# Pablete1234/parquet-floor

Measured on AMD Instinct MI355X. Metric: decoded GB/s + rows/s (node), lineitem-shape Snappy+dict, 1/2/4/8 GPUs, higher is better.
Workload: dtype u8; 1 GPU; lineitem SF1 x1 (6001215 rows x 1, 16 cols, 6 row groups of 1Mi rows), Snappy + dictionary, device-resident; row_groups_per_rank=6, compressed_page_bytes_rank0=217870360

## Files before the change

### parquet-floor_amd/csrc/pf_internal.h

```cpp
#pragma once
#include <stdint.h>

#ifdef __HIPCC__
#define PF_HD __host__ __device__
#else
#define PF_HD
#endif

namespace pf {

struct Int2 {
    int x, y;
};

struct PfOpts {
    int exec = 5;
    bool ba_fused = true;
    bool page_null = false;
    int null_stagger = 0;
    bool nest_timeout = false;
    uint32_t null_dcap = 0;
    unsigned debug_skip = 0;
    int force_serial = 0;
    int force_redo = 0;
    bool zc = true;
    bool dl_kernel = true;
    bool h2d_kernel = false;
    int h2d_grid = 256;
    bool dl_stream = true;
    bool dl_prio = false;
    bool debug_plan = false;
    int64_t nest_seg = 0;
    bool nest_seg_set = false;
    bool dbp_par = true;
    bool bloom_first = true;
    int fix_shift = 1;
};

constexpr uint32_t FBLK = 4096;
constexpr uint32_t BA_TILE = 8192;
constexpr uint64_t BA_SHORT = 48;
constexpr uint32_t STICKY_DICT = 64u << 10;
constexpr uint32_t SNAP_RB = 128;
constexpr uint32_t SNAP_WIN = 64 * SNAP_RB;
constexpr uint32_t SNAP_WWORDS = SNAP_WIN / 32;
constexpr uint32_t SNAP_BLOCK = 65536;

struct SnapWin {
    uint32_t entry;
    uint32_t exit;
    uint32_t out;
    uint32_t flags;
};

struct SnapEnt {
    uint32_t pos;
    uint32_t out;
};

enum : int32_t {
    PG_V2 = 1,
    PG_COMPRESSED = 2,
    PG_DICT = 4,
};

struct SnappyJob {
    const uint8_t* src;
    uint8_t* dst;
    uint32_t src_len;
    uint32_t dst_len;
    int32_t page;
    int32_t chunk;
    uint32_t split_base;
    uint32_t n_pieces;
    uint32_t* tokmap;
    uint32_t win_base;
    uint32_t n_win;
    uint8_t* ddst;
    uint32_t dlo;
    uint32_t dgran;
    uint32_t dflags;
    uint32_t lit;
};

struct ZstdJob {
    const uint8_t* src;
    uint8_t* dst;
    uint32_t src_len;
    uint32_t dst_len;
    int32_t page;
    int32_t chunk;
    uint32_t exact;
    uint32_t produced;
};
constexpr int ZSTD_GRID = 512;
constexpr uint32_t ZSTD_LIT_MAX = 128u << 10;
PF_HD inline uint32_t zstd_lit_stride(uint32_t max_dst) {
    return ((max_dst < ZSTD_LIT_MAX ? max_dst : ZSTD_LIT_MAX) + 255u) / 256u * 256u + 256u;
}

enum : int32_t { DONE_FIXED = 1, DONE_FLAT = 2, DONE_NULL = 4, DONE_PAGE = 8 };

enum : int32_t { DIRECT_NONE = 0, DIRECT_VALUES = 1, DIRECT_INPLACE = 2 };

struct DevPage {
    const uint8_t* body;
    const uint8_t* lvl;
    uint32_t body_len;
    uint32_t rep_len;
    uint32_t def_len;
    int32_t chunk;
    int32_t flags;
    int32_t encoding;
    int32_t def_enc;
    int32_t rep_enc;
    int32_t num_values;
    int32_t done;
    int64_t entry_start;
    int64_t n_slots;
    int64_t n_values;
    int64_t n_rows;
    int64_t n_chars;
    int64_t slot_start;
    int64_t value_start;
    int64_t row_start;
    int64_t char_start;
    uint32_t* aux;
    int64_t aux_cap;
    int32_t ba_job;
    int32_t counted;
    uint32_t* runtab;
    uint32_t* lvltab;
    uint32_t lvl_cap;
    uint64_t* dx;
    int64_t dx_total;
    int64_t dx_bad;
    uint32_t dx_data;
    uint32_t dx_pad;
    const int* jfb;
    int32_t direct;
    int32_t direct_pad;
    uint8_t* seg;
    int32_t nseg;
    int32_t seg_len;
    int32_t seg_ok;
    int32_t nwin;
    struct WinPub* npub;
    uint8_t* dbp;
    struct WinPub* dbp_pub;
    int32_t dbp_nwin;
    int32_t dbp_ok;
    uint32_t dbp_bcap;
    uint32_t dbp_pad;
};
// ... 160 lines not shown
```

### parquet-floor_amd/csrc/pf_launch.h

```cpp
#pragma once
#include <hip/hip_runtime.h>

#include "pf_internal.h"
#include "pfloor.h"

namespace pf {

void launch_snappy_serial(const SnappyJob* d_jobs, int n_jobs, const int* d_fallback, DevChunkResult* d_res, hipStream_t s);
void launch_snappy_parse(const SnappyJob* d_jobs, int n_jobs, const int2* d_wins, int n_wins, SnapWin* d_win, SnapEnt* d_ent,
                         uint32_t* d_lane_out, uint32_t* d_splits, int* d_fb, int max_nwin, hipStream_t s);
void launch_snappy_exec(const SnappyJob* d_jobs, int n_jobs, const int2* d_pieces, int n_pieces, uint32_t* d_splits, int* d_fb,
                        DevChunkResult* d_res, int exec, hipStream_t s);
void launch_snappy(const SnappyJob* d_jobs, int n_jobs, const int2* d_wins, int n_wins, SnapWin* d_win, SnapEnt* d_ent,
                   uint32_t* d_lane_out, const int2* d_pieces, int n_pieces, uint32_t* d_splits, int* d_fb,
                   DevChunkResult* d_res, int max_nwin, int exec, hipStream_t s);

void launch_zstd(ZstdJob* d_jobs, const int* d_order, int n_jobs, uint8_t* d_lit, uint32_t lit_stride, DevChunkResult* d_res,
                 hipStream_t s);

void launch_snappy_head(SnappyJob* d_jobs, int n_jobs, DevPage* d_pages, const DevChunk* d_chunks, int* d_fb,
                        const DevChunkResult* d_res, hipStream_t st);
void launch_snappy_litcopy(const SnappyJob* d_jobs, const int* d_list, int n, const int* d_fb, hipStream_t st);

void launch_ba(BaJob* d_jobs, int n_jobs, const int2* d_tiles, int n_tiles, DevChunkResult* d_res, hipStream_t st,
               bool short_values);

void launch_runs(const DevChunk* d_chunks, DevPage* d_pages, const int* d_list, int n, DevChunkResult* d_res, hipStream_t st);
void launch_lvl(const DevChunk* d_chunks, DevPage* d_pages, const int* d_list, int n, DevChunkResult* d_res, hipStream_t st,
                bool page_null, NullCaps nc);
void launch_count_flat(const DevChunk* d_chunks, DevPage* d_pages, const int* d_list, int n, int n_flat, const int2* d_dblk,
                       int n_dblk, DevChunkResult* d_res, BaJob* d_bajobs, hipStream_t st);
void launch_flat(const DevChunk* d_chunks, DevPage* d_pages, const int* d_list, int nfix, int n, int n4, int n8, int* d_fbq,
                 DevChunkResult* d_res, hipStream_t st, NullCaps nc, int stagger);

void launch_nest_lvl(const DevChunk* d_chunks, DevPage* d_pages, const int* d_list, int n, int max_nwin, DevChunkResult* d_res,
                     hipStream_t st, bool force_timeout);
void launch_count(const DevChunk* d_chunks, DevPage* d_pages, const int* d_list, int n, DevChunkResult* d_res, BaJob* d_bajobs,
                  hipStream_t st, int idle_grid);
void launch_nest_count(const DevChunk* d_chunks, DevPage* d_pages, const int* d_list, int n, const int2* d_segs, int n_segs,
                       DevChunkResult* d_res, hipStream_t st);
void launch_scan(DevChunk* d_chunks, DevPage* d_pages, const int* d_list, int n, DevChunkResult* d_res, uint8_t* arena,
                 uint64_t cap, unsigned long long* used, hipStream_t st);
void launch_decode(const DevChunk* d_chunks, DevPage* d_pages, const int* d_list, int n, int n_first, DevChunkResult* d_res,
                   hipStream_t st, int idle_grid);
void launch_nest_decode(const DevChunk* d_chunks, DevPage* d_pages, const int2* d_segs, int n_segs, DevChunkResult* d_res,
                        hipStream_t st);

void launch_delta(const DevChunk* d_chunks, DevPage* d_pages, const int* d_list, int n, int max_dbp_nwin, DevChunkResult* d_res,
                  hipStream_t st);
void launch_dlen(const DevChunk* d_chunks, DevPage* d_pages, const int* d_list, int n, DevChunkResult* d_res, hipStream_t st);
void launch_dba_chars(const DevChunk* d_chunks, DevPage* d_pages, const int* d_list, int n, DevChunkResult* d_res, hipStream_t st);

void launch_window(const DevChunk* d_chunks, const DevChunkResult* d_res, const DevWin* d_wins, DevWinRes* d_wres, int n_wins,
                   int copy_grid, const uint8_t* chars_base, uint8_t* wchars_base, int64_t out_delta, int64_t bits_delta,
                   hipStream_t st);

struct SelBufs {
    DevSelHead* head;
    DevSelChunk* sc;
    const DevPred* preds;
    const uint8_t* blob;
    const int32_t* win_of;
    uint64_t* mask;
    uint32_t* tile_count;
    uint32_t* tile_base;
    int32_t* rows;
    uint32_t* ba_sum;
    uint32_t* ba_base;
    int64_t* ba_total;
    int64_t rows_cap, tiles_cap;
    int32_t n_preds;
};
void launch_filter(const DevChunk* d_chunks, const DevChunkResult* d_res, const DevWinRes* d_wres, const SelBufs& f, int n_chunks,
                   int gather_grid, const uint8_t* chars_base, uint8_t* wchars_base, int64_t out_delta, int64_t bits_delta,
                   hipStream_t st);

void launch_page_scan(const ScanChunk* d_chunks, int n_chunks, pf_page_desc* d_pages, ScanCrc* d_crcs, ScanResult* d_res,
                      hipStream_t s);
void launch_page_crc(const ScanCrc* d_crcs, const int* d_list, int n, ScanResult* d_res, int32_t* d_bad, hipStream_t s);

}
```

### parquet-floor_amd/csrc/pf_pages.hip

```cpp
#include <hip/hip_runtime.h>

#include "pf_launch.h"
#include "pf_pages.h"
#include "pf_snappy_par.h"

namespace pf {

#ifdef PF_STAMPS
__device__ unsigned long long pf_pstamps[16];
#define PSTAMP(i, v) atomicAdd(&pf_pstamps[i], (unsigned long long)(v))
extern "C" int pf_debug_pstamps(unsigned long long* out, int n, int reset) {
    if (hipMemcpyFromSymbol(out, HIP_SYMBOL(pf_pstamps), sizeof(unsigned long long) * (n < 16 ? n : 16)) != hipSuccess) return -1;
    if (reset) {
        unsigned long long z[16] = {};
        if (hipMemcpyToSymbol(HIP_SYMBOL(pf_pstamps), z, sizeof z) != hipSuccess) return -1;
    }
    return 0;
}
#else
#define PSTAMP(i, v) ((void)0)
#endif

#ifndef PF_FT
#define PF_FT 2048
#endif
constexpr int FT = PF_FT;
constexpr int FEPT = FT / NT;
static_assert(FT <= int(FBLK) && FBLK % FT == 0 && FEPT <= 32, "tiles divide blocks; a thread's entries fit a 32-bit mask");
#ifndef PF_FTX
#define PF_FTX 2048
#endif
constexpr int FTX = PF_FTX;
constexpr int FEPTX = FTX / NT;
static_assert(FTX <= int(FBLK) && FBLK % FTX == 0, "fixed-width tiles divide blocks");
#ifndef PF_RUN_CAP
#define PF_RUN_CAP 256
#endif
constexpr int RUN_CAP = PF_RUN_CAP;
constexpr uint32_t DSTR_CAP = 256;

__global__ __launch_bounds__(128) void k_runs(const DevChunk* __restrict__ chunks, DevPage* pages,
                                              const int* __restrict__ list, DevChunkResult* res) {
    __shared__ Run R[RUN_CAP];
    __shared__ int s_allp, s_nr, s_res;
    __shared__ uint32_t s_cov;
    const int pi = list[blockIdx.x];
    DevPage& pg = pages[pi];
    uint32_t* T = pg.runtab;
    if (!T) return;
    const DevChunk& ck = chunks[pg.chunk];
    const int tid = threadIdx.x;
    Sections s;
    if (res[pg.chunk].status != 0 || !page_sections(pg, ck, s) || s.val_n == 0 || s.val[0] > 32) {
        if (tid == 0) T[3] = 0;
// ... 560 lines not shown
                    if (R.packed) {
                        const uint64_t bit = uint64_t(R.data) + uint64_t(e - R.first) * uint64_t(id_bw);
                        id = (bit >> 3) + 12 <= ids_n ? bits_fast(ids + (bit >> 3), uint32_t(bit & 7), id_bw)
                                                      : bits_le(ids, ids_n, bit, id_bw);
                    }
                    if (int64_t(id) >= ck.dict_n) { bad = 1; continue; }
                    const uint8_t* src = ck.dict_data + uint64_t(id) * uint64_t(w);
                    if (w == 8 && dalign) *reinterpret_cast<uint64_t*>(dst) = *reinterpret_cast<const uint64_t*>(src);
                    else if (w == 4 && dalign) *reinterpret_cast<uint32_t*>(dst) = *reinterpret_cast<const uint32_t*>(src);
                    else copy_value(dst, src, w);
                } else if (boolean) {
                    if ((e >> 3) >= s.val_n) { bad = 1; continue; }
                    dst[0] = uint8_t((s.val[e >> 3] >> (e & 7)) & 1u);
                } else if (enc == 0) {
                    if ((uint64_t(e) + 1) * uint64_t(w) > s.val_n) { bad = 1; continue; }
                    const uint8_t* src = s.val + uint64_t(e) * uint64_t(w);
                    if (w == 8 && src + 12 <= vend) *reinterpret_cast<uint64_t*>(dst) = gld_u64_12(src);
                    else if (w == 4 && src + 8 <= vend) *reinterpret_cast<uint32_t*>(dst) = gld_u32_8(src);
                    else copy_value(dst, src, w);
                } else {
                    const uint64_t* dv = reinterpret_cast<const uint64_t*>(pg.aux);
                    if (w == 8) *reinterpret_cast<uint64_t*>(dst) = dv[e];
                    else *reinterpret_cast<uint32_t*>(dst) = uint32_t(dv[e]);
                }
            }
        }
        if (ck.max_def > 0 && ck.validity) {
            const uint64_t b0 = slot_base + e0, b1 = b0 + want;
            uint32_t* vw = reinterpret_cast<uint32_t*>(ck.validity);
            for (uint64_t wd = (b0 >> 5) + tid; wd <= ((b1 - 1) >> 5); wd += NT) {
                const uint64_t lo = max(b0, wd << 5), hi = min(b1, (wd + 1) << 5);
                const uint32_t m = uint32_t((hi - lo >= 32 ? 0xffffffffull : ((1ull << (hi - lo)) - 1ull)) << (lo & 31));
                if (lo == (wd << 5) && hi == ((wd + 1) << 5)) vw[wd] = m;
                else atomicOr(vw + wd, m);
            }
        }
        if (__syncthreads_or(bad)) return 1;
    }
    return 0;
}

__device__ __forceinline__ bool flat_fixed_block(FixedLds& S, const DevChunk* __restrict__ chunks, DevPage* pages, const int2 pbk,
                                 DevChunkResult* res) {
    if (pbk.x < 0) return true;
    const int pi = pbk.x;
    const uint32_t blk = uint32_t(pbk.y) & 0x0fffffffu;
    const uint32_t bsz = FBLK << (uint32_t(pbk.y) >> 28);
    DevPage& pg = pages[pi];
    const DevChunk& ck = chunks[pg.chunk];
    const int tid = threadIdx.x;
    const int* jfb = pg.jfb;
    const bool dval = pg.direct == DIRECT_VALUES;
    const int jf = jfb != nullptr ? *jfb : FB_WHOLE + 1;
    if ((res[pg.chunk].status != 0) | (ck.max_rep != 0) | (ck.ptype == 6) | ((pg.done & DONE_NULL) != 0)) return false;
    if (dval & (jf <= FB_WHOLE)) {
        const uint32_t ne = uint32_t(pg.num_values), e_begin = blk * bsz;
        if (e_begin >= ne && blk > 0) return true;
        const uint32_t e_end = min(ne, e_begin + bsz);
        if (ck.max_def > 0 && ck.validity && e_end > e_begin) {
            const uint64_t b0 = uint64_t(pg.entry_start) + e_begin, b1 = uint64_t(pg.entry_start) + e_end;
            uint32_t* vw = reinterpret_cast<uint32_t*>(ck.validity);
            for (uint64_t wd = (b0 >> 5) + threadIdx.x; wd <= ((b1 - 1) >> 5); wd += NT) {
                const uint64_t lo = max(b0, wd << 5), hi = min(b1, (wd + 1) << 5);
                const uint32_t m = uint32_t((hi - lo >= 32 ? 0xffffffffull : ((1ull << (hi - lo)) - 1ull)) << (lo & 31));
                if (lo == (wd << 5) && hi == ((wd + 1) << 5)) vw[wd] = m;
                else atomicOr(vw + wd, m);
            }
        }
        if (threadIdx.x == 0) {
            if (ck.needs_count == 0)
                atomicAdd(reinterpret_cast<unsigned long long*>(&res[pg.chunk].num_values), (unsigned long long)(e_end - e_begin));
            atomicOr(&pg.done, DONE_FIXED);
        }
        return true;
    }
    Sections s;
    if (!page_sections(pg, ck, s)) return false;
    const int enc = pg.encoding;
    const bool boolean = ck.ptype == 0, dict = is_dict_enc(enc);
    const int w = ck.width;
    bool take = ck.max_def == 0 || s.def_rle;
    if (enc == 0) {
    } else if (dict) take = take && !boolean;
    else if (enc == 5) take = take && (ck.ptype == 1 || ck.ptype == 2) && pg.aux != nullptr;
    else take = false;
    if (!take) return false;
    const uint32_t ne = uint32_t(pg.num_values);
    if (blk > 0 && blk * bsz >= ne) return true;
    const int id_bw = (dict && s.val_n > 0) ? int(s.val[0]) : 0;
    const uint8_t* ids = dict && s.val_n > 0 ? s.val + 1 : s.val;
    const uint64_t ids_n = dict && s.val_n > 0 ? s.val_n - 1 : 0;
    const uint32_t* T = pg.runtab;
    uint32_t t0 = 0, t3 = 0;
    if (T != nullptr) { t0 = T[0]; t3 = T[3]; }
    const bool tab = (t3 == 1u) & (t0 <= uint32_t(RUN_CAP));
    if (tid == 0)
        S.allp = tab ? 1 : (ck.max_def == 0 ? 1 : all_present(s.def, s.def_n, bit_width(ck.max_def), ne, uint32_t(ck.max_def)));
    __syncthreads();
    if (!S.allp) return false;
    const uint32_t e_begin = blk * bsz;
    const uint32_t e_end = min(ne, e_begin + bsz);
#ifdef PF_STAMPS
    const unsigned long long ft0 = __builtin_amdgcn_s_memtime();
#endif
    if (dict) {
        if (tab) {
            const uint32_t nr = T[0], cov = T[1];
// ... 5 lines not shown
                r.count = nf - r.first;
                r.data = T[5 + 2 * i];
                r.packed = f >> 31;
                S.vrun[i] = r;
            }
            if (tid == 0) { S.nvrun = int(nr); S.vcover = cov; S.vlo = 0; S.vres = cov >= ne ? 0 : 1; }
        } else if (tid < 64) {
            if (tid == 0) { S.nvrun = 0; S.vcover = 0; S.vres = 0; S.vlo = e_begin; S.vst = RunWalk{0, 0}; }
            if (s.val_n > 0 && id_bw <= 32) {
                const int rr = wave_walk_runs(ids, ids_n, id_bw, e_begin, e_end, S.vrun, RUN_CAP, S.nvrun, S.vcover, S.vst, RunWalk{0, 0});
                if (tid == 0) S.vres = rr;
            }
        }
        __syncthreads();
    }
    const bool direct = dval & (jf <= FB_WHOLE);
    const int err = flat_present_fixed(S, ck, pg, s, dict, boolean, enc, w, ids, ids_n, id_bw,
                                       uint64_t(pg.entry_start), e_begin, e_end, direct);
#ifdef PF_STAMPS
    if (tid == 0) { const unsigned long long dt_ = __builtin_amdgcn_s_memtime() - ft0; PSTAMP(1, dt_); PSTAMP(0, 1); atomicMax(&pf_pstamps[9], dt_); }
#endif
    if (tid == 0) {
        if (err) set_status(res, pg.chunk, ST_CORRUPT, pi);
        else if (ck.needs_count == 0)
            atomicAdd(reinterpret_cast<unsigned long long*>(&res[pg.chunk].num_values), (unsigned long long)(e_end - e_begin));
        atomicOr(&pg.done, DONE_FIXED);
    }
    return true;
}

__device__ __forceinline__ void null_fallback(int* fbq, int2 pbk) {
    if (threadIdx.x == 0) reinterpret_cast<int2*>(fbq + 4)[atomicAdd(fbq, 1)] = pbk;
}

#ifndef PF_FIXED_OCC
#define PF_FIXED_OCC 6
#endif
__global__ __launch_bounds__(NT, PF_FIXED_OCC) void k_flat_fixed(const DevChunk* __restrict__ chunks, DevPage* pages,
                                                              const int2* __restrict__ blocks, DevChunkResult* res, int* fbq) {
    __shared__ FixedLds S;
    const int2 pbk = blocks[blockIdx.x];
    if (!flat_fixed_block(S, chunks, pages, pbk, res)) null_fallback(fbq, pbk);
}

__device__ __forceinline__ void flat_block(FlatLds& S, const DevChunk* __restrict__ chunks, DevPage* pages, const int2 pbk,
                           DevChunkResult* res) {
    if (pbk.x < 0) return;
    const int pi = pbk.x;
    const uint32_t blk = uint32_t(pbk.y) & 0x0fffffffu;
    const uint32_t bsz = FBLK << (uint32_t(pbk.y) >> 28);
    DevPage& pg = pages[pi];
    const DevChunk& ck = chunks[pg.chunk];
    const int tid = threadIdx.x;
    if ((res[pg.chunk].status != 0) | (ck.max_rep != 0) | ((pg.done & (DONE_FIXED | DONE_NULL)) != 0)) return;
    Sections s;
    if (!page_sections(pg, ck, s)) return;
    const int enc = pg.encoding;
    const bool binary = ck.ptype == 6, boolean = ck.ptype == 0, dict = is_dict_enc(enc);
    const int w = ck.width;
    bool take = ck.max_def == 0 || s.def_rle;
    if (enc == 0) {
    } else if (dict) take = take && !boolean;
    else if (enc == 5) take = take && (ck.ptype == 1 || ck.ptype == 2) && pg.aux != nullptr;
    else take = false;
    if (!take) return;

    const int bwd = bit_width(ck.max_def);
    const uint32_t ne = uint32_t(pg.num_values);
    const int id_bw = (dict && s.val_n > 0) ? int(s.val[0]) : 0;
    const uint8_t* ids = dict && s.val_n > 0 ? s.val + 1 : s.val;
    const uint64_t ids_n = dict && s.val_n > 0 ? s.val_n - 1 : 0;
    const bool counted = ck.needs_count != 0;
    const uint64_t slot_base = uint64_t(pg.entry_start);
    if (blk > 0 && blk * bsz >= ne) return;
    const uint32_t* T = pg.runtab;
    uint32_t t0 = 0, t3 = 0;
    if (T != nullptr) { t0 = T[0]; t3 = T[3]; }
    const bool tab = (t3 == 1u) & (t0 <= uint32_t(RUN_CAP));
    if (tid == 0) S.allp = tab ? 1 : (ck.max_def == 0 ? 1 : all_present(s.def, s.def_n, bwd, ne, uint32_t(ck.max_def)));
    __syncthreads();
    const bool split = S.allp;
    if (!split && blk > 0) return;
    const uint32_t e_begin = split ? blk * bsz : 0u;
    const uint32_t e_end = split ? min(ne, e_begin + bsz) : ne;
#ifdef PF_STAMPS
    const unsigned long long ft0 = __builtin_amdgcn_s_memtime();
    if (tid == 0) { PSTAMP(0, 1); if (dict) PSTAMP(6, 1); if (binary) PSTAMP(7, 1); }
#endif
    if (tid < 64) {
        if (tid == 0) { S.ndrun = 0; S.dcover = ne; S.dres = 0; S.dst = RunWalk{0, 0}; }
        if (!split && ck.max_def > 0) {
            const int rr = wave_walk_runs(s.def, s.def_n, bwd, 0, ne, S.drun, RUN_CAP, S.ndrun, S.dcover, S.dst, RunWalk{0, 0});
            if (tid == 0) S.dres = rr;
        }
    } else if (tid < 128 && !(split && tab)) {
        if (tid == 64) { S.nvrun = 0; S.vcover = 0; S.vres = 0; S.vlo = e_begin; S.vst = RunWalk{0, 0}; }
        if (dict && s.val_n > 0 && id_bw <= 32) {
            const int rr = wave_walk_runs(ids, ids_n, id_bw, e_begin, split ? e_end : ne, S.vrun, RUN_CAP, S.nvrun,
                                          S.vcover, S.vst, RunWalk{0, 0});
            if (tid == 64) S.vres = rr;
        }
    }
    if (split && tab) {
        const uint32_t nr = T[0], cov = T[1];
        for (uint32_t i = tid; i < nr; i += NT) {
            const uint32_t f = T[4 + 2 * i];
            const uint32_t nf = i + 1 < nr ? (T[4 + 2 * (i + 1)] & 0x7fffffffu) : cov;
// ... 194 lines not shown
                if (eb + k >= want) continue;
                if ((fv >> k) & 1u) {
                    S.coff[vo + j] = c;
                    S.csrc[vo + j] = my_src[k];
                    c += my_len[k];
                    j++;
                }
                ck.offsets[slot_base + e0 + eb + k + 1] = int32_t(char_base + c);
            }
        }
        if (ck.max_def > 0 && fv) {
            const uint64_t abase = (slot_base + e0) & ~uint64_t(31);
            const uint64_t rb = slot_base + e0 + eb - abase;
            const uint32_t sh = uint32_t(rb & 31);
            atomicOr(&S.vbits[rb >> 5], fv << sh);
            if (sh + FEPT > 32 && sh) atomicOr(&S.vbits[(rb >> 5) + 1], fv >> (32 - sh));
        }
        __syncthreads();
#ifdef PF_STAMPS
        { const unsigned long long t_ = __builtin_amdgcn_s_memtime(); if (tid == 0) { PSTAMP(4, t_ - ft1); PSTAMP(3, 1); PSTAMP(14, t_ - fs_); } ft1 = t_; fs_ = t_; }
#endif
        if (binary) {
            const uint8_t* sb = dict ? ck.dict_data : s.val;
            const uint8_t* se = dict ? pages[ck.dict_page].body + pages[ck.dict_page].body_len : s.val + s.val_n;
            if (tchars <= SHORT_AVG * tv) copy_chars_short(S.coff, S.csrc, tv, tchars, sb, ck.chars + char_base);
            else if (!dict) copy_chars_plain(S.coff, S.csrc, tv, tchars, sb, se, ck.chars + char_base, S.cv);
            else copy_chars_fast(S.coff, S.csrc, tv, tchars, sb, se, ck.chars + char_base, S.cv);
        }
        FSTAMP(15);
        if (ck.max_def > 0 && ck.validity) flush_bits(S.vbits, slot_base + e0, want, ck.validity);
        vidx += tv;
        char_base += tchars;
        __syncthreads();
#ifdef PF_STAMPS
        { const unsigned long long t_ = __builtin_amdgcn_s_memtime(); if (tid == 0) PSTAMP(5, t_ - ft1); ft1 = t_; }
#endif
    }
#ifdef PF_STAMPS
    if (tid == 0) {
        const unsigned long long dt_ = __builtin_amdgcn_s_memtime() - ft0;
        PSTAMP(1, dt_);
        atomicMax(&pf_pstamps[binary ? 8 : 9], dt_);
        if (!split) PSTAMP(10, 1);
    }
#endif
    if (tid == 0) {
        if (err) set_status(res, pg.chunk, ST_CORRUPT, pi);
        else if (!counted) atomicAdd(reinterpret_cast<unsigned long long*>(&res[pg.chunk].num_values),
                                     (unsigned long long)(vidx - e_begin));
        atomicOr(&pg.done, DONE_FLAT);
    }
}


#ifndef PF_FLAT_OCC
#define PF_FLAT_OCC 5
#endif
__global__ __launch_bounds__(NT, PF_FLAT_OCC) void k_flat_all(const DevChunk* __restrict__ chunks, DevPage* pages,
                                                 const int2* __restrict__ blocks, int n, const int* __restrict__ fbq,
                                                 DevChunkResult* res) {
    __shared__ union FlatAllLds {
        FixedLds f;
        FlatLds g;
    } S;
    if (int(blockIdx.x) >= n) {
        const int nq = fbq[0], g = int(gridDim.x) - n;
        for (int i = int(blockIdx.x) - n; i < nq; i += g) {
            const int2 pq = reinterpret_cast<const int2*>(fbq + 4)[i];
            if (!flat_fixed_block(S.f, chunks, pages, pq, res)) {
                __syncthreads();
                flat_block(S.g, chunks, pages, pq, res);
            }
            __syncthreads();
        }
        return;
    }
    const int2 pbk = blocks[blockIdx.x];
    if (flat_fixed_block(S.f, chunks, pages, pbk, res)) return;
    __syncthreads();
    flat_block(S.g, chunks, pages, pbk, res);
}

constexpr uint32_t LVL_STAGE = 4096;

__device__ __forceinline__ uint32_t lds_bits(const uint8_t* st, uint32_t bit, uint32_t k) {
    const uint32_t* w = reinterpret_cast<const uint32_t*>(st);
    const uint32_t wi = bit >> 5, sh = bit & 31u;
    const uint64_t v = uint64_t(w[wi]) | (uint64_t(w[wi + 1]) << 32);
    return uint32_t(v >> sh) & (k >= 32 ? 0xffffffffu : ((1u << k) - 1u));
}

__device__ __forceinline__ uint32_t lvl_run_at(const uint32_t* runs, uint32_t nr, uint32_t e) {
    uint32_t lo = 0, hi = nr;
    while (hi - lo > 1) {
        const uint32_t m = (lo + hi) >> 1;
        if (runs[4 * m] <= e) lo = m; else hi = m;
    }
    return lo;
}
__device__ inline uint32_t lvl_values_before(const uint32_t* runs, uint32_t r, uint32_t e, const uint8_t* stage,
                                             uint32_t woff, int bw, uint32_t maxd) {
    const uint32_t first = runs[4 * r], data = runs[4 * r + 1], cw = runs[4 * r + 2];
    const uint32_t before = e - first;
    uint32_t vb = runs[4 * r + 3];
    if (!(cw >> 31)) return vb + (data == maxd ? before : 0u);
    if (bw == 1) {
// ... 910 lines not shown
    }
    __syncthreads();
    const int r = wave_walk_runs(p, n, bw, lo, limit, R, cap, s_nr, s_cov, s_st, RunWalk{pos0, first0});
    __syncthreads();
    if (tid == 0) {
        o2[0] = uint32_t(r); o2[1] = uint32_t(s_nr); o2[2] = s_cov; o2[3] = uint32_t(s_st.pos); o2[4] = s_st.first;
    }
    for (int i = tid; i < s_nr; i += 64) { o2[5 + 4 * i] = R[i].first; o2[6 + 4 * i] = R[i].count; o2[7 + 4 * i] = R[i].data; o2[8 + 4 * i] = R[i].packed; }
}

extern "C" int pf_debug_walk_runs(const uint8_t* stream, uint64_t n, int bw, uint32_t lo, uint32_t limit, int cap,
                                  uint32_t pos0, uint32_t first0, uint32_t* out) {
    if (cap > int(RUN_CAP) || cap < 0) return -1;
    uint8_t* d = nullptr;
    uint32_t* o = nullptr;
    const size_t ob = 4 * size_t(2 * (5 + 4 * cap));
    if (hipMalloc(&d, n + 64) != hipSuccess) return -1;
    if (hipMalloc(&o, ob) != hipSuccess) { (void)hipFree(d); return -1; }
    int rc = 0;
    if (hipMemset(d, 0, n + 64) != hipSuccess || hipMemcpy(d, stream, n, hipMemcpyHostToDevice) != hipSuccess ||
        hipMemset(o, 0, ob) != hipSuccess)
        rc = -1;
    if (!rc) {
        hipLaunchKernelGGL(k_debug_walk, dim3(1), dim3(64), 0, 0, d, n, bw, lo, limit, cap, pos0, first0, o);
        if (hipDeviceSynchronize() != hipSuccess || hipMemcpy(out, o, ob, hipMemcpyDeviceToHost) != hipSuccess) rc = -1;
    }
    (void)hipFree(d);
    (void)hipFree(o);
    return rc;
}
#endif

void launch_count_flat(const DevChunk* d_chunks, DevPage* d_pages, const int* d_list, int n, int n_flat, const int2* d_dblk,
                       int n_dblk, DevChunkResult* d_res, BaJob* d_bajobs, hipStream_t st) {
    if (n <= 0) return;
    if (n_dblk > 0) hipLaunchKernelGGL(k_count_dict, dim3(n_dblk), dim3(NT), 0, st, d_chunks, d_pages, d_dblk, d_res);
    if (n_flat > 0) hipLaunchKernelGGL(k_count_flat, dim3(n_flat), dim3(NT), 0, st, d_chunks, d_pages, d_list, d_res, d_bajobs);
}
void launch_runs(const DevChunk* d_chunks, DevPage* d_pages, const int* d_list, int n, DevChunkResult* d_res,
                 hipStream_t st) {
    if (n > 0) hipLaunchKernelGGL(k_runs, dim3(n), dim3(128), 0, st, d_chunks, d_pages, d_list, d_res);
}
void launch_lvl(const DevChunk* d_chunks, DevPage* d_pages, const int* d_list, int n, DevChunkResult* d_res,
                hipStream_t st, bool page_null, NullCaps nc) {
    if (n <= 0) return;
#ifdef PF_DIAG
    if (page_null) hipLaunchKernelGGL(k_page_null, dim3(n), dim3(PN_NT), 0, st, d_chunks, d_pages, d_list, d_res);
#else
    (void)page_null;
#endif
    hipLaunchKernelGGL(k_lvl, dim3(n), dim3(LT_NT), 0, st, d_chunks, d_pages, d_list, d_res, nc.dcap, nc.icap);
}
void launch_flat(const DevChunk* d_chunks, DevPage* d_pages, const int* d_list, int nfix, int n, int n4, int n8, int* d_fbq,
                 DevChunkResult* d_res, hipStream_t st, NullCaps nc, int stagger) {
    const int2* blocks = reinterpret_cast<const int2*>(d_list);
    const size_t dyn = size_t(nc.dcap) + 32u + nc.icap + 32u + nc.dlds;
    if (n4 > 0)
        hipLaunchKernelGGL(k_flat_null<4>, dim3(n4), dim3(NTN), dyn, st, d_chunks, d_pages, blocks + nfix + n, d_res, nc, stagger, d_fbq);
    if (n8 > 0)
        hipLaunchKernelGGL(k_flat_null<8>, dim3(n8), dim3(NTN), dyn, st, d_chunks, d_pages, blocks + nfix + n + n4, d_res, nc, stagger,
                           d_fbq);
    if (nfix > 0) hipLaunchKernelGGL(k_flat_fixed, dim3(nfix), dim3(NT), 0, st, d_chunks, d_pages, blocks, d_res, d_fbq);
    const int nq = nfix + n4 + n8;
    const int nqw = nq < 32 ? nq : 32;
    if (n + nqw > 0)
        hipLaunchKernelGGL(k_flat_all, dim3(n + nqw), dim3(NT), 0, st, d_chunks, d_pages, blocks + nfix, n, d_fbq, d_res);
}

}
```

### parquet-floor_amd/csrc/pf_runtime.hip

```cpp
#include <hip/hip_runtime.h>

#include <algorithm>
#include <chrono>
#include <cstdio>
#include <cstdlib>
#include <cstring>
#include <memory>
#include <mutex>
#include <string>
#include <vector>

#include "pf_ctx.h"
#include "pf_host.h"
#include "pf_launch.h"
#include "pf_plan.h"
#include "pf_snappy_par.h"
#include "pfloor.h"

using namespace pf;

static_assert(sizeof(Int2) == sizeof(int2) && alignof(Int2) <= alignof(int2), "the planner's pairs are the kernels' int2");

namespace {

// ... 81 lines not shown
    uint32_t* d_splits = reinterpret_cast<uint32_t*>(meta + p.off_splits);
    int* d_fallback = reinterpret_cast<int*>(meta + p.off_fallback);
    const int2* d_wins = reinterpret_cast<const int2*>(meta + p.off_wins);

#ifdef PF_DIAG
    const unsigned skip = ctx->opts.debug_skip;
#else
    constexpr unsigned skip = 0;
#endif
    if (!ctx->meta_by_kernel) {
        if (p.bits_bytes) HIPCHK(ctx, hipMemsetAsync(ctx->d_bits.p, 0, p.bits_bytes, st));
        if (p.npub_bytes) HIPCHK(ctx, hipMemsetAsync(static_cast<uint8_t*>(ctx->d_scratch.p) + p.off_npub, 0, p.npub_bytes, st));
    }
    EVREC(ctx, ctx->ev[1], st);
    if (!(skip & 1u)) launch_snappy_head(d_jobs, n_jobs, d_pages, d_chunks, d_fallback, d_res, st);
    if (!(skip & 1u)) launch_snappy_litcopy(d_jobs, list(L_DJOBS), len(L_DJOBS), d_fallback, st);
    if (!(skip & 1u)) launch_snappy_parse(d_jobs, n_jobs, d_wins, int(p.snap.wins.size()), p.snap.d_win, p.snap.d_ent,
                        p.snap.d_lane_out, d_splits, d_fallback, p.snap.max_snap_win, st);
    EVREC(ctx, ctx->ev[2], st);
    if (!(skip & 2u))
        launch_snappy_exec(d_jobs, n_jobs, d_pieces, int(p.snap.pieces.size()), d_splits, d_fallback, d_res, ctx->opts.exec, st);
    launch_zstd(reinterpret_cast<ZstdJob*>(meta + p.off_zjobs), list(L_ZSTD), int(p.zjobs.size()),
                static_cast<uint8_t*>(ctx->d_scratch.p) + p.off_zlit, p.zlit_stride, d_res, st);
    EVREC(ctx, ctx->ev[3], st);
    BaJob* d_bajobs = reinterpret_cast<BaJob*>(meta + p.off_bajobs);
    const int2* d_batiles = reinterpret_cast<const int2*>(meta + p.off_batiles);
    const int n_ba = int(p.bajobs.size()), n_bt = int(p.ba_tiles.size());
    if (!(skip & 4u)) launch_ba(d_bajobs, p.n_ba_dict, d_batiles, p.n_ba_dict_tiles, d_res, st, p.ba_short_dict && ctx->opts.ba_fused);
    EVREC(ctx, ctx->ev[4], st);
    launch_delta(d_chunks, d_pages, list(L_DELTA), len(L_DELTA), p.max_dbp_nwin, d_res, st);
    EVREC(ctx, ctx->ev[5], st);
    if (!(skip & 8u)) launch_runs(d_chunks, d_pages, list(L_RUNS), len(L_RUNS), d_res, st);
    NullCaps ncaps = p.null_caps;
    if (ctx->opts.null_dcap) ncaps.dcap = ctx->opts.null_dcap;
    if (!(skip & 8u)) launch_lvl(d_chunks, d_pages, list(L_LVL), len(L_LVL), d_res, st, ctx->opts.page_null, ncaps);
    launch_dlen(d_chunks, d_pages, list(L_DLEN), len(L_DLEN), d_res, st);
    EVREC(ctx, ctx->ev[6], st);
    launch_nest_lvl(d_chunks, d_pages, list(L_NEST), n_nest, p.max_nwin, d_res, st, ctx->opts.nest_timeout);
    if (!(skip & 16u)) {
        launch_count_flat(d_chunks, d_pages, list(L_COUNT), len(L_COUNT), p.n_count_flat, pairs(L_CDICT), len(L_CDICT) / 2,
                          d_res, d_bajobs, st);
        launch_count(d_chunks, d_pages, list(L_COUNT), len(L_COUNT), d_res, d_bajobs, st, COUNT_IDLE_GRID);
    }
    launch_nest_count(d_chunks, d_pages, list(L_NEST), n_nest, pairs(L_NSEG), n_nseg, d_res, st);
    if (!(skip & 4u))
        launch_ba(d_bajobs + p.n_ba_dict, n_ba - p.n_ba_dict, d_batiles + p.n_ba_dict_tiles, n_bt - p.n_ba_dict_tiles,
                  d_res, st, p.ba_short_data && ctx->opts.ba_fused);
    EVREC(ctx, ctx->ev[7], st);
    launch_scan(d_chunks, d_pages, list(L_SCAN), len(L_SCAN), d_res, static_cast<uint8_t*>(ctx->d_chars.p),
                ctx->d_chars.cap, used, st);
    EVREC(ctx, ctx->ev[8], st);
    if (!(skip & 32u))
        launch_flat(d_chunks, d_pages, list(L_FLAT), p.n_flat_fixed, p.n_flat_all, p.n_null4, p.n_null8,
                    reinterpret_cast<int*>(meta + p.off_nfbq), d_res, st, ncaps, ctx->opts.null_stagger);
    EVREC(ctx, ctx->ev[9], st);
    if (!(skip & 64u)) launch_decode(d_chunks, d_pages, list(L_DECODE), len(L_DECODE), p.n_decode_first, d_res, st, DECODE_IDLE_GRID);
    launch_nest_decode(d_chunks, d_pages, pairs(L_NSEG), n_nseg, d_res, st);
    launch_dba_chars(d_chunks, d_pages, list(L_DBA), len(L_DBA), d_res, st);
    EVREC(ctx, ctx->ev[10], st);
    if (!ctx->wins.empty()) {
        const int nw = int(ctx->wins.size());
        const size_t res_off = align_up(sizeof(DevWin) * nw, 256);
        DevWin* d_wins = static_cast<DevWin*>(ctx->d_win.p);
        DevWinRes* d_wres = reinterpret_cast<DevWinRes*>(static_cast<uint8_t*>(ctx->d_win.p) + res_off);
        EVREC(ctx, ctx->ev_win[0], st);
        launch_window(d_chunks, d_res, d_wins, d_wres, nw, ctx->win_grid, static_cast<const uint8_t*>(ctx->d_chars.p),
                      static_cast<uint8_t*>(ctx->d_wchars.p),
                      static_cast<uint8_t*>(ctx->d_wout.p) - static_cast<uint8_t*>(ctx->d_out.p),
                      static_cast<uint8_t*>(ctx->d_wbits.p) - static_cast<uint8_t*>(ctx->d_bits.p), st);
        EVREC(ctx, ctx->ev_win[1], st);
        HIPCHK(ctx, hipMemcpyAsync(static_cast<uint8_t*>(ctx->h_win.p) + res_off, d_wres, sizeof(DevWinRes) * nw,
                                   hipMemcpyDeviceToHost, st));
    }
    if (ctx->filtered()) {
        const DevWinRes* d_wres = ctx->wins.empty() ? nullptr : reinterpret_cast<const DevWinRes*>(
            static_cast<const uint8_t*>(ctx->d_win.p) + align_up(sizeof(DevWin) * ctx->wins.size(), 256));
        EVREC(ctx, ctx->ev_sel[0], st);
        launch_filter(d_chunks, d_res, d_wres, ctx->sel, ctx->n_chunks, ctx->sel_grid, static_cast<const uint8_t*>(ctx->d_chars.p),
                      static_cast<uint8_t*>(ctx->d_wchars.p),
                      static_cast<uint8_t*>(ctx->d_wout.p) - static_cast<uint8_t*>(ctx->d_out.p),
                      static_cast<uint8_t*>(ctx->d_wbits.p) - static_cast<uint8_t*>(ctx->d_bits.p), st);
        EVREC(ctx, ctx->ev_sel[1], st);
        HIPCHK(ctx, hipMemcpyAsync(ctx->h_sel.p, ctx->d_sel.p, ctx->sel_up_off, hipMemcpyDeviceToHost, st));
    }
    HIPCHK(ctx, hipGetLastError());
    const size_t res_pad = align_up(sizeof(DevChunkResult) * ctx->n_chunks, 256);
    if (ctx->zc && ctx->h_res.d) {
        copy_words(ctx->h_res.d, meta + p.off_res, sizeof(DevChunkResult) * ctx->n_chunks,
                   static_cast<uint8_t*>(ctx->h_res.d) + res_pad, d_chunks, sizeof(DevChunk) * ctx->n_chunks, st);
    } else {
        HIPCHK(ctx, hipMemcpyAsync(ctx->h_res.p, meta + p.off_res, sizeof(DevChunkResult) * ctx->n_chunks,
                                   hipMemcpyDeviceToHost, st));
        HIPCHK(ctx, hipMemcpyAsync(static_cast<uint8_t*>(ctx->h_res.p) + res_pad, d_chunks, sizeof(DevChunk) * ctx->n_chunks,
                                   hipMemcpyDeviceToHost, st));
    }
    HIPCHK(ctx, hipEventRecord(ctx->ev_done, st));
    return PF_OK;
}

int upload_meta(pf_ctx* ctx) {
    const BatchPlan& p = ctx->plan;
    uint8_t* h = static_cast<uint8_t*>(ctx->h_meta.p);
    auto put = [&](size_t off, const auto& v) { if (!v.empty()) std::memcpy(h + off, v.data(), sizeof(v[0]) * v.size()); };
    std::memset(h, 0, p.meta_bytes);
    put(p.off_chunks, p.chunks);
    put(p.off_pages, p.pages);
    put(p.off_jobs, p.jobs);
// ... 57 lines not shown
    return PF_OK;
}

}



extern "C" {

int pf_abi_version(void) { return PF_ABI_VERSION; }

const char* pf_last_error(pf_ctx* ctx) { return ctx ? ctx->err.c_str() : g_err.c_str(); }

int pf_device_count(int* count) {
    if (!count) return fail(nullptr, PF_ERR_INVALID_ARG, "null count");
    int n = 0;
    hipError_t e = hipGetDeviceCount(&n);
    if (e != hipSuccess) { *count = 0; return fail(nullptr, PF_ERR_HIP, hipGetErrorString(e)); }
    *count = n;
    return PF_OK;
}

namespace {
#ifdef PF_DIAG
void opts_from_env(pf::PfOpts& o) {
    auto on = [](const char* name, bool dflt) { const char* e = std::getenv(name); return e ? e[0] == '1' : dflt; };
    auto num = [](const char* name, int dflt) { const char* e = std::getenv(name); return e ? std::atoi(e) : dflt; };
    o.exec = num("PF_EXEC", o.exec);
    o.ba_fused = on("PF_BA_FUSED", o.ba_fused);
    o.page_null = on("PF_PAGE_NULL", o.page_null);
    o.nest_timeout = on("PF_DEBUG_NEST_TIMEOUT", o.nest_timeout);
    o.null_dcap = uint32_t(std::max(0, num("PF_NULL_DCAP", 0))) & ~15u;
    o.null_stagger = num("PF_DEBUG_NULL_STAGGER", o.null_stagger);
    if (const char* e = std::getenv("PF_DEBUG_SKIP")) {
        const char* names[] = {"parse", "exec", "ba", "levels", "count", "flat", "decode"};
        for (int i = 0; i < 7; i++)
            if (std::strstr(e, names[i])) o.debug_skip |= 1u << i;
    }
    o.force_serial = num("PF_DEBUG_FORCE_SERIAL", o.force_serial);
    o.force_redo = num("PF_DEBUG_FORCE_REDO", o.force_redo);
    o.zc = on("PF_ZC", o.zc);
    o.dl_kernel = on("PF_DL_KERNEL", o.dl_kernel);
    o.dl_stream = on("PF_DL_STREAM", o.dl_stream);
    o.h2d_kernel = on("PF_H2D_KERNEL", o.h2d_kernel);
    o.h2d_grid = std::max(1, num("PF_H2D_GRID", o.h2d_grid));
    o.dl_prio = on("PF_DL_PRIO", o.dl_prio);
    o.debug_plan = on("PF_DEBUG_PLAN", o.debug_plan);
    if (const char* e = std::getenv("PF_NEST_SEG")) {
        o.nest_seg = std::atoll(e);
        o.nest_seg_set = true;
    }
    o.dbp_par = on("PF_DBP_PAR", o.dbp_par);
    o.bloom_first = on("PF_BLOOM_FIRST", o.bloom_first);
    const int fb = num("PF_FIX_BLK", 8192);
    o.fix_shift = fb >= 16384 ? 2 : (fb >= 8192 ? 1 : 0);
}
#endif

int ctx_init(pf_ctx* ctx, pf_ctx* peer) {
#ifdef PF_DIAG
    opts_from_env(ctx->opts);
#endif
    HIPCHK(nullptr, hipSetDevice(ctx->device));
    if (peer) {
        ctx->streams = peer->streams;
    } else {
        ctx->streams = std::make_shared<Streams>();
        ctx->streams->device = ctx->device;
        HIPCHK(nullptr, hipStreamCreateWithFlags(&ctx->streams->stream, hipStreamNonBlocking));
    }
    ctx->stream = ctx->streams->stream;
    ctx->zc = ctx->opts.zc;
    HIPCHK(nullptr, hipEventCreateWithFlags(&ctx->ev_done, hipEventDisableTiming));
    HIPCHK(nullptr, hipEventCreateWithFlags(&ctx->ev_copy, hipEventDisableTiming));
    HIPCHK(nullptr, hipEventCreateWithFlags(&ctx->ev_dl, hipEventDisableTiming));
    for (auto& e : ctx->ev) HIPCHK(nullptr, hipEventCreate(&e));
    for (auto& e : ctx->ev_bloom) HIPCHK(nullptr, hipEventCreate(&e));
    for (auto& e : ctx->ev_win) HIPCHK(nullptr, hipEventCreate(&e));
    for (auto& e : ctx->ev_sel) HIPCHK(nullptr, hipEventCreate(&e));
    return PF_OK;
}

int ctx_create(int device, pf_ctx* peer, pf_ctx** out) {
    pf_ctx* ctx = new pf_ctx();
    ctx->device = device;
    const int rc = ctx_init(ctx, peer);
    if (rc != PF_OK) {
        const std::string msg = g_err;
        pf_ctx_destroy(ctx);
        g_err = msg;
        return rc;
    }
    *out = ctx;
    return PF_OK;
}
}

int pf_ctx_create(int device, pf_ctx** out) {
    if (!out) return fail(nullptr, PF_ERR_INVALID_ARG, "null out");
    *out = nullptr;
    int n = 0;
    if (hipGetDeviceCount(&n) != hipSuccess || device < 0 || device >= n)
        return fail(nullptr, PF_ERR_INVALID_ARG, "no such HIP device");
    return ctx_create(device, nullptr, out);
}

// ... 911 lines not shown
```

Measured before the change: 374.7 decoded GB/s.

## Add block-parallel dictionary-string decode kernel staging dict and ids in LDS

Adds a k_flat_dstr kernel that decodes dictionary-encoded byte-array pages with small dictionaries per 4096-entry block. It stages the run table, the dictionary bytes and the packed id window in shared memory, computes offsets with a block scan, and gathers chars through an LDS window with aligned 16-byte stores. Pages it handles are marked DONE_DSTR so the generic flat and decode paths skip them. This is meant to replace slower generic string decoding for low-cardinality string columns, at the cost of a large LDS footprint and a fallback path whenever the dictionary or string lengths exceed the caps.

```diff
diff --git a/parquet-floor_amd/csrc/pf_dstr_ids.h b/parquet-floor_amd/csrc/pf_dstr_ids.h
--- /dev/null
+++ b/parquet-floor_amd/csrc/pf_dstr_ids.h
@@ -0,0 +1,53 @@
+#pragma once
+#include <stdint.h>
+
+#include "pf_internal.h"
+
+namespace pf {
+
+PF_HD inline uint32_t dstr_run_at(const uint32_t* rt, uint32_t nr, uint32_t e) {
+    uint32_t lo = 0, hi = nr;
+    while (hi - lo > 1) {
+        const uint32_t m = (lo + hi) >> 1;
+        if ((rt[2 * m] & 0x7fffffffu) <= e) lo = m; else hi = m;
+    }
+    return lo;
+}
+
+template <class Words>
+PF_HD inline void dstr_ids16(const uint32_t* rt, uint32_t nr, uint32_t cov, uint32_t e0, uint32_t n, int bw, int64_t bias,
+                             const Words& W, uint32_t (&id)[16]) {
+    const uint64_t mask = bw >= 32 ? 0xffffffffull : ((1ull << bw) - 1ull);
+    uint32_t r = nr ? dstr_run_at(rt, nr, e0) : 0u;
+    uint32_t first = 0, end = 0, data = 0, packed = 0;
+    if (nr) {
+        const uint32_t f = rt[2 * r];
+        first = f & 0x7fffffffu;
+        packed = f >> 31;
+        data = rt[2 * r + 1];
+        end = r + 1 < nr ? (rt[2 * r + 2] & 0x7fffffffu) : cov;
+    }
+#ifdef __HIP_DEVICE_COMPILE__
+    #pragma unroll
+#endif
+    for (uint32_t k = 0; k < 16; k++) {
+        id[k] = 0;
+        const uint32_t e = e0 + k;
+        if (k >= n || e >= cov || nr == 0) continue;
+        while (e >= end && r + 1 < nr) {
+            r++;
+            const uint32_t f = rt[2 * r];
+            first = f & 0x7fffffffu;
+            packed = f >> 31;
+            data = rt[2 * r + 1];
+            end = r + 1 < nr ? (rt[2 * r + 2] & 0x7fffffffu) : cov;
+        }
+        if (!packed || bw == 0) { id[k] = packed ? 0u : data; continue; }
+        const uint64_t fb = uint64_t(int64_t(uint64_t(data) + uint64_t(e - first) * uint64_t(bw)) + bias);
+        const uint32_t wi = uint32_t(fb >> 5), sh = uint32_t(fb & 31u);
+        const uint64_t x = (uint64_t(W(wi)) | (uint64_t(W(wi + 1u)) << 32)) >> sh;
+        id[k] = uint32_t(x & mask);
+    }
+}
+
+}
diff --git a/parquet-floor_amd/csrc/pf_internal.h b/parquet-floor_amd/csrc/pf_internal.h
--- a/parquet-floor_amd/csrc/pf_internal.h
+++ b/parquet-floor_amd/csrc/pf_internal.h
@@ -34,6 +34,7 @@
     bool nest_seg_set = false;
     bool dbp_par = true;
     bool bloom_first = true;
+    bool flat_dstr = true;
     int fix_shift = 1;
 };
 
@@ -99,7 +100,7 @@
     return ((max_dst < ZSTD_LIT_MAX ? max_dst : ZSTD_LIT_MAX) + 255u) / 256u * 256u + 256u;
 }
 
-enum : int32_t { DONE_FIXED = 1, DONE_FLAT = 2, DONE_NULL = 4, DONE_PAGE = 8 };
+enum : int32_t { DONE_FIXED = 1, DONE_FLAT = 2, DONE_NULL = 4, DONE_PAGE = 8, DONE_DSTR = 16 };
 
 enum : int32_t { DIRECT_NONE = 0, DIRECT_VALUES = 1, DIRECT_INPLACE = 2 };
 
diff --git a/parquet-floor_amd/csrc/pf_launch.h b/parquet-floor_amd/csrc/pf_launch.h
--- a/parquet-floor_amd/csrc/pf_launch.h
+++ b/parquet-floor_amd/csrc/pf_launch.h
@@ -31,7 +31,7 @@
 void launch_count_flat(const DevChunk* d_chunks, DevPage* d_pages, const int* d_list, int n, int n_flat, const int2* d_dblk,
                        int n_dblk, DevChunkResult* d_res, BaJob* d_bajobs, hipStream_t st);
 void launch_flat(const DevChunk* d_chunks, DevPage* d_pages, const int* d_list, int nfix, int n, int n4, int n8, int* d_fbq,
-                 DevChunkResult* d_res, hipStream_t st, NullCaps nc, int stagger);
+                 const int2* d_dblk, int n_dblk, DevChunkResult* d_res, hipStream_t st, NullCaps nc, int stagger);
 
 void launch_nest_lvl(const DevChunk* d_chunks, DevPage* d_pages, const int* d_list, int n, int max_nwin, DevChunkResult* d_res,
                      hipStream_t st, bool force_timeout);
diff --git a/parquet-floor_amd/csrc/pf_pages.hip b/parquet-floor_amd/csrc/pf_pages.hip
--- a/parquet-floor_amd/csrc/pf_pages.hip
+++ b/parquet-floor_amd/csrc/pf_pages.hip
@@ -1,5 +1,6 @@
 #include <hip/hip_runtime.h>
 
+#include "pf_dstr_ids.h"
 #include "pf_launch.h"
 #include "pf_pages.h"
 #include "pf_snappy_par.h"
@@ -666,7 +667,9 @@
     const int* jfb = pg.jfb;
     const bool dval = pg.direct == DIRECT_VALUES;
     const int jf = jfb != nullptr ? *jfb : FB_WHOLE + 1;
-    if ((res[pg.chunk].status != 0) | (ck.max_rep != 0) | (ck.ptype == 6) | ((pg.done & DONE_NULL) != 0)) return false;
+    const int done = pg.done;
+    if (done & DONE_DSTR) return true;
+    if ((res[pg.chunk].status != 0) | (ck.max_rep != 0) | (ck.ptype == 6) | ((done & DONE_NULL) != 0)) return false;
     if (dval & (jf <= FB_WHOLE)) {
         const uint32_t ne = uint32_t(pg.num_values), e_begin = blk * bsz;
         if (e_begin >= ne && blk > 0) return true;
@@ -778,7 +781,7 @@
     DevPage& pg = pages[pi];
     const DevChunk& ck = chunks[pg.chunk];
     const int tid = threadIdx.x;
-    if ((res[pg.chunk].status != 0) | (ck.max_rep != 0) | ((pg.done & (DONE_FIXED | DONE_NULL)) != 0)) return;
+    if ((res[pg.chunk].status != 0) | (ck.max_rep != 0) | ((pg.done & (DONE_FIXED | DONE_NULL | DONE_DSTR)) != 0)) return;
     Sections s;
     if (!page_sections(pg, ck, s)) return;
     const int enc = pg.encoding;
@@ -1079,6 +1082,240 @@
     }
 }
 
+#ifndef PF_DSTR_LMAX
+#define PF_DSTR_LMAX 32
+#endif
+#ifndef PF_DSTR_DICT
+#define PF_DSTR_DICT 4096
+#endif
+#ifndef PF_DSTR_WIN
+#define PF_DSTR_WIN 16384
+#endif
+#ifndef PF_DSTR_OCC
+#define PF_DSTR_OCC 6
+#endif
+constexpr uint32_t DSTR_LMAX = PF_DSTR_LMAX, DSTR_DICT = PF_DSTR_DICT, DSTR_WIN = PF_DSTR_WIN;
+static_assert(DSTR_WIN % 16 == 0 && DSTR_DICT % 16 == 0 && DSTR_DICT + 16 < 65536 && DSTR_LMAX < 65536,
+              "{pos, len} of a staged dictionary value share one word");
+static_assert(RUN_CAP <= NT && int(DSTR_CAP) <= NT && FBLK == 16u * NT, "one run, one dictionary value, 16 entries per thread");
+struct DstrLds {
+    uint32_t rt[2 * RUN_CAP];
+    uint32_t dpl[DSTR_CAP];
+    u32x4 dict[DSTR_DICT / 16 + 2];
+    u32x4 win[DSTR_WIN / 16 + 2];
+    uint32_t scan_tmp[NT / 64];
+    uint32_t wlo[NT / 64], whi[NT / 64];
+};
+#ifdef PF_DIAG
+__device__ unsigned long long pf_dstr_counts[2];
+extern "C" int pf_debug_dstr_counts(unsigned long long* out, int reset) {
+    if (hipMemcpyFromSymbol(out, HIP_SYMBOL(pf_dstr_counts), sizeof(unsigned long long) * 2) != hipSuccess) return -1;
+    if (reset) {
+        const unsigned long long z[2] = {0, 0};
+        if (hipMemcpyToSymbol(HIP_SYMBOL(pf_dstr_counts), z, sizeof z) != hipSuccess) return -1;
+    }
+    return 0;
+}
+#define DSTR_COUNT(i) (threadIdx.x == 0 ? (void)atomicAdd(&pf_dstr_counts[i], 1ull) : (void)0)
+#else
+#define DSTR_COUNT(i) ((void)0)
+#endif
+
+__device__ __forceinline__ u32x4 ld16_within(uintptr_t a, uintptr_t beg, uintptr_t end) {
+    if (a >= beg && a + 16u <= end) return *reinterpret_cast<const PF_GLOBAL u32x4*>(a);
+    uint32_t q[4] = {0, 0, 0, 0};
+    #pragma unroll
+    for (uint32_t b = 0; b < 16u; b++)
+        if (a + b >= beg && a + b < end) q[b >> 2] |= uint32_t(*reinterpret_cast<const PF_GLOBAL uint8_t*>(a + b)) << (8 * (b & 3));
+    return u32x4{q[0], q[1], q[2], q[3]};
+}
+
+template <int LEAD>
+__device__ __forceinline__ void store_offs16(int32_t* p, const uint32_t (&o)[16]) {
+    #pragma unroll
+    for (int k = 0; k < LEAD; k++) p[k] = int32_t(o[k]);
+    #pragma unroll
+    for (int k = LEAD; k + 4 <= 16; k += 4) *reinterpret_cast<u32x4*>(p + k) = u32x4{o[k], o[k + 1], o[k + 2], o[k + 3]};
+    #pragma unroll
+    for (int k = LEAD + (16 - LEAD) / 4 * 4; k < 16; k++) p[k] = int32_t(o[k]);
+}
+
+__global__ __launch_bounds__(NT, PF_DSTR_OCC) void k_flat_dstr(const DevChunk* __restrict__ chunks, DevPage* pages,
+                                                            const int2* __restrict__ blocks, DevChunkResult* res) {
+    __shared__ DstrLds S;
+    const int2 pb = blocks[blockIdx.x];
+    const int pi = pb.x;
+    const uint32_t blk = uint32_t(pb.y);
+    DevPage& pg = pages[pi];
+    const DevChunk& ck = chunks[pg.chunk];
+    const int tid = threadIdx.x;
+    const uint32_t ne = uint32_t(pg.num_values);
+    const uint32_t b0 = blk * FBLK;
+    if (blk > 0 && b0 >= ne) return;
+    bool ok = (res[pg.chunk].status == 0) & (ck.max_rep == 0) & (ck.ptype == 6) & is_dict_enc(pg.encoding) & (pg.counted == 1) &
+              (pg.num_values > 0) & (ck.dict_n > 0) & (ck.dict_n <= int64_t(DSTR_CAP)) & (ck.dict_page >= 0);
+    ok = ok && ck.dict_pos != nullptr && ck.dict_len != nullptr && ck.dict_data != nullptr && ck.chars != nullptr &&
+         ck.offsets != nullptr;
+    Sections s;
+    ok = ok && page_sections(pg, ck, s) && count_dict_page(pg, ck, s) && s.val[0] <= 32;
+    const uintptr_t dbeg = reinterpret_cast<uintptr_t>(ck.dict_data);
+    uintptr_t dend = dbeg;
+    if (ok) {
+        const DevPage& dp = pages[ck.dict_page];
+        dend = reinterpret_cast<uintptr_t>(dp.body) + dp.body_len;
+        ok = dend > dbeg && dend - dbeg <= uintptr_t(DSTR_DICT);
+    }
+    if (!ok) {
+        if (blk == 0) DSTR_COUNT(1);
+        return;
+    }
+    const uint32_t b1 = min(ne, b0 + FBLK);
+    const uint32_t* T = pg.runtab;
+    const uint32_t nr = T[0], cov = T[1];
+    const uint32_t dn = uint32_t(ck.dict_n), dbytes = uint32_t(dend - dbeg);
+    const int id_bw = int(s.val[0]);
+    const uint8_t* ids = s.val + 1;
+    const uint64_t ids_n = s.val_n - 1;
+    const uint64_t bc_blk = blk > 0 ? flat_block_chars(pg)[blk] : 0ull;
+    int bad = 0;
+    uint32_t mylo = 0xffffffffu, myhi = 0u;
+    if (uint32_t(tid) < nr) {
+        const uint32_t f = T[4 + 2 * tid], d = T[5 + 2 * tid];
+        const uint32_t nf = uint32_t(tid) + 1 < nr ? (T[6 + 2 * tid] & 0x7fffffffu) : cov;
+        S.rt[2 * tid] = f;
+        S.rt[2 * tid + 1] = d;
+        const uint32_t first = f & 0x7fffffffu;
+        const uint32_t a = max(first, b0), z = min(nf, b1);
+        if ((f >> 31) && a < z) {
+            mylo = uint32_t((uint64_t(d) + uint64_t(a - first) * uint64_t(id_bw)) >> 3);
+            myhi = uint32_t((uint64_t(d) + uint64_t(z - first) * uint64_t(id_bw) + 7u) >> 3);
+        }
+    }
+    const uint32_t doff = uint32_t(dbeg & 15u);
+    if (uint32_t(tid) < dn) {
+        const uint32_t pos = gptr(ck.dict_pos)[tid], len = gptr(ck.dict_len)[tid];
+        bad = (len > DSTR_LMAX) | (pos > dbytes) | (len > dbytes - min(pos, dbytes));
+        S.dpl[tid] = (doff + pos) | (len << 16);
+    }
+    for (uint32_t c = tid; c < (doff + dbytes + 15u) / 16u; c += NT) S.dict[c] = ld16_within(dbeg - doff + 16u * c, dbeg, dend);
+    #pragma unroll
+    for (int d = 32; d >= 1; d >>= 1) {
+        mylo = min(mylo, uint32_t(__shfl_xor(mylo, d, 64)));
+        myhi = max(myhi, uint32_t(__shfl_xor(myhi, d, 64)));
+    }
+    if ((tid & 63) == 0) { S.wlo[tid >> 6] = mylo; S.whi[tid >> 6] = myhi; }
+    if (__syncthreads_or(bad)) {
+        if (blk == 0) DSTR_COUNT(1);
+        return;
+    }
+    uint32_t lo = 0xffffffffu, hi = 0u;
+    #pragma unroll
+    for (int w = 0; w < NT / 64; w++) { lo = min(lo, S.wlo[w]); hi = max(hi, S.whi[w]); }
+    const uintptr_t ibeg = reinterpret_cast<uintptr_t>(ids), iend = ibeg + ids_n;
+    const uintptr_t ia0 = (ibeg + (lo < hi ? lo : 0u)) & ~uintptr_t(15);
+    const uint32_t inb = lo < hi ? (uint32_t(ibeg + hi - ia0) + 8u + 15u) & ~15u : 0u;
+    const bool ilds = inb > 0 && inb <= uint32_t(sizeof(S.win));
+    if (ilds) {
+        for (uint32_t c = tid; c < inb / 16u; c += NT) S.win[c] = ld16_within(ia0 + 16u * c, ibeg, iend);
+        __syncthreads();
+    }
+    const int64_t bias = ilds ? 8 * (int64_t(ibeg) - int64_t(ia0)) : 0;
+    const uint32_t* const wl = reinterpret_cast<const uint32_t*>(S.win);
+    const auto W = [&](uint32_t w) -> uint32_t {
+        if (ilds) return wl[w];
+        return ld32le(ids, uint64_t(w) * 4u, ids_n);
+    };
+    const uint32_t e0 = b0 + 16u * uint32_t(tid);
+    const uint32_t n = e0 < b1 ? min(16u, b1 - e0) : 0u;
+    uint32_t pl[16];
+    uint32_t lsum = 0;
+    {
+        uint32_t id[16];
+        dstr_ids16(S.rt, nr, cov, e0, n, id_bw, bias, W, id);
+        #pragma unroll
+        for (uint32_t k = 0; k < 16; k++) {
+            pl[k] = 0;
+            if (k >= n) continue;
+            if (id[k] >= dn) { bad = 1; continue; }
+            pl[k] = S.dpl[id[k]];
+            lsum += pl[k] >> 16;
+        }
+    }
+    uint32_t tot;
+    const uint32_t lo_c = block_excl_scan<NT>(lsum, S.scan_tmp, tot);
+    const uint64_t char_base = uint64_t(pg.char_start) + bc_blk;
+    if (char_base + tot > uint64_t(pg.char_start + pg.n_chars)) bad = 1;
+    if (__syncthreads_or(bad)) {
+        if (tid == 0) {
+            set_status(res, pg.chunk, ST_CORRUPT, pi);
+            atomicOr(&pg.done, DONE_DSTR | DONE_FLAT);
+        }
+        return;
+    }
+    const uint64_t slot_base = uint64_t(pg.entry_start);
+    if (n > 0) {
+        uint32_t o[16];
+        uint32_t c = uint32_t(char_base) + lo_c;
+        #pragma unroll
+        for (uint32_t k = 0; k < 16; k++) { c += pl[k] >> 16; o[k] = c; }
+        int32_t* op = ck.offsets + slot_base + e0 + 1;
+        if (n == 16) {
+            switch ((4u - uint32_t((reinterpret_cast<uintptr_t>(op) >> 2) & 3u)) & 3u) {
+                case 0: store_offs16<0>(op, o); break;
+                case 1: store_offs16<1>(op, o); break;
+                case 2: store_offs16<2>(op, o); break;
+                default: store_offs16<3>(op, o); break;
+            }
+        } else {
+            #pragma unroll
+            for (uint32_t k = 0; k < 16; k++) if (k < n) op[k] = int32_t(o[k]);
+        }
+    }
+    if (ck.max_def > 0 && ck.validity) {
+        const uint64_t v0 = slot_base + b0, v1 = slot_base + b1;
+        uint32_t* vw = reinterpret_cast<uint32_t*>(ck.validity);
+        for (uint64_t wd = (v0 >> 5) + tid; wd <= ((v1 - 1) >> 5); wd += NT) {
+            const uint64_t l = max(v0, wd << 5), h = min(v1, (wd + 1) << 5);
+            const uint32_t m = uint32_t((h - l >= 32 ? 0xffffffffull : ((1ull << (h - l)) - 1ull)) << (l & 31));
+            if (l == (wd << 5) && h == ((wd + 1) << 5)) vw[wd] = m;
+            else atomicOr(vw + wd, m);
+        }
+    }
+    const uintptr_t gout = reinterpret_cast<uintptr_t>(ck.chars + char_base);
+    const uint32_t a0c = uint32_t(gout & 15u);
+    const uintptr_t g0 = gout - a0c;
+    const uint32_t vend = a0c + tot, my0 = a0c + lo_c;
+    uint8_t* const w8 = reinterpret_cast<uint8_t*>(S.win);
+    const uint8_t* const d8 = reinterpret_cast<const uint8_t*>(S.dict);
+    for (uint32_t w0 = 0; w0 < vend && tot > 0; w0 += DSTR_WIN) {
+        const uint32_t w1 = min(vend, w0 + DSTR_WIN);
+        if (w0 > 0) __syncthreads();
+        if (my0 < w1 && my0 + lsum > w0) {
+            uint32_t v = my0;
+            #pragma unroll
+            for (uint32_t k = 0; k < 16; k++) {
+                const uint32_t len = pl[k] >> 16, pos = pl[k] & 0xffffu;
+                const uint32_t s0 = max(v, w0), s1 = min(v + len, w1);
+                for (uint32_t b = s0; b < s1; b++) w8[b - w0] = d8[pos + (b - v)];
+                v += len;
+            }
+        }
+        __syncthreads();
+        for (uint32_t ci = tid; ci < (w1 - w0 + 15u) / 16u; ci += NT) {
+            const uint32_t vp = w0 + 16u * ci;
+            if (vp >= a0c && vp + 16u <= vend) {
+                *reinterpret_cast<PF_GLOBAL u32x4*>(g0 + vp) = S.win[ci];
+            } else {
+                for (uint32_t b = 0; b < 16u; b++)
+                    if (vp + b >= a0c && vp + b < vend) reinterpret_cast<uint8_t*>(g0 + vp)[b] = w8[16u * ci + b];
+            }
+        }
+    }
+    if (tid == 0) {
+        atomicOr(&pg.done, DONE_DSTR | DONE_FLAT);
+        DSTR_COUNT(0);
+    }
+}
 
 #ifndef PF_FLAT_OCC
 #define PF_FLAT_OCC 5
@@ -2095,7 +2332,7 @@
     hipLaunchKernelGGL(k_lvl, dim3(n), dim3(LT_NT), 0, st, d_chunks, d_pages, d_list, d_res, nc.dcap, nc.icap);
 }
 void launch_flat(const DevChunk* d_chunks, DevPage* d_pages, const int* d_list, int nfix, int n, int n4, int n8, int* d_fbq,
-                 DevChunkResult* d_res, hipStream_t st, NullCaps nc, int stagger) {
+                 const int2* d_dblk, int n_dblk, DevChunkResult* d_res, hipStream_t st, NullCaps nc, int stagger) {
     const int2* blocks = reinterpret_cast<const int2*>(d_list);
     const size_t dyn = size_t(nc.dcap) + 32u + nc.icap + 32u + nc.dlds;
     if (n4 > 0)
@@ -2104,6 +2341,7 @@
         hipLaunchKernelGGL(k_flat_null<8>, dim3(n8), dim3(NTN), dyn, st, d_chunks, d_pages, blocks + nfix + n + n4, d_res, nc, stagger,
                            d_fbq);
     if (nfix > 0) hipLaunchKernelGGL(k_flat_fixed, dim3(nfix), dim3(NT), 0, st, d_chunks, d_pages, blocks, d_res, d_fbq);
+    if (n_dblk > 0) hipLaunchKernelGGL(k_flat_dstr, dim3(n_dblk), dim3(NT), 0, st, d_chunks, d_pages, d_dblk, d_res);
     const int nq = nfix + n4 + n8;
     const int nqw = nq < 32 ? nq : 32;
     if (n + nqw > 0)
diff --git a/parquet-floor_amd/csrc/pf_runtime.hip b/parquet-floor_amd/csrc/pf_runtime.hip
--- a/parquet-floor_amd/csrc/pf_runtime.hip
+++ b/parquet-floor_amd/csrc/pf_runtime.hip
@@ -157,7 +157,8 @@
     EVREC(ctx, ctx->ev[8], st);
     if (!(skip & 32u))
         launch_flat(d_chunks, d_pages, list(L_FLAT), p.n_flat_fixed, p.n_flat_all, p.n_null4, p.n_null8,
-                    reinterpret_cast<int*>(meta + p.off_nfbq), d_res, st, ncaps, ctx->opts.null_stagger);
+                    reinterpret_cast<int*>(meta + p.off_nfbq), pairs(L_CDICT), ctx->opts.flat_dstr ? len(L_CDICT) / 2 : 0, d_res, st,
+                    ncaps, ctx->opts.null_stagger);
     EVREC(ctx, ctx->ev[9], st);
     if (!(skip & 64u)) launch_decode(d_chunks, d_pages, list(L_DECODE), len(L_DECODE), p.n_decode_first, d_res, st, DECODE_IDLE_GRID);
     launch_nest_decode(d_chunks, d_pages, pairs(L_NSEG), n_nseg, d_res, st);
@@ -321,6 +322,7 @@
     }
     o.dbp_par = on("PF_DBP_PAR", o.dbp_par);
     o.bloom_first = on("PF_BLOOM_FIRST", o.bloom_first);
+    o.flat_dstr = on("PF_FLAT_DSTR", o.flat_dstr);
     const int fb = num("PF_FIX_BLK", 8192);
     o.fix_shift = fb >= 16384 ? 2 : (fb >= 8192 ? 1 : 0);
 }
```

New measurement: 391.5 decoded GB/s, median of 6. 4.5% higher.
